# liuQuan98/APR

Measured on AMD Instinct MI355X. Metric: point-cloud pairs/sec (120k-pt KITTI frame, FCGF encode+match+SVD), higher is better.
Workload: dtype f32

## Files before the change

apr_amd/_lib.py:

```python
from __future__ import annotations

import ctypes as C
import os

import torch

_HERE = os.path.dirname(os.path.abspath(__file__))
LIB_PATH = os.path.join(_HERE, "lib", "libapr_hip.so")

_p = C.c_void_p
_i32, _i64, _u64, _f32, _f64, _sz = C.c_int32, C.c_int64, C.c_uint64, C.c_float, C.c_double, C.c_size_t

class PairDesc(C.Structure):
    _fields_ = [("f0", C.c_void_p), ("n0", C.c_int64), ("f1", C.c_void_p), ("n1", C.c_int64),
                ("xyz0", C.c_void_p), ("xyz1", C.c_void_p), ("seed", C.c_uint64)]


class SpconvDesc(C.Structure):
    _fields_ = [("inp", C.c_void_p), ("ldi", C.c_int64), ("nbr", C.c_void_p), ("n_out", C.c_int64),
                ("K", C.c_int32), ("cin", C.c_int32), ("cout", C.c_int32), ("relu", C.c_int32),
                ("w_packed", C.c_void_p), ("scale", C.c_void_p), ("shift", C.c_void_p),
                ("residual", C.c_void_p), ("ldr", C.c_int64), ("out", C.c_void_p), ("ldo", C.c_int64),
                ("counters", C.c_void_p), ("plist", C.c_void_p), ("prod_scratch", C.c_void_p),
                ("plist_bytes", C.c_int64), ("w_bf3", C.c_void_p),
# ... 63 lines not shown
    "apr_map_scratch_bytes": (_sz, [_i64]),
    "apr_voxelize": (C.c_int, [_p, _i64, _f32, _i32, _p, _p]),
    "apr_map_build": (C.c_int, [_p, _i64, _p, _i32, _p, _p, _i64, _p, _p, _p, _p, _p, _sz, _p]),
    "apr_kernel_map_transpose": (C.c_int, [_p, _i64, _i32, _i64, _p, _p]),
    "apr_voxelize_segments": (C.c_int, [_p, _i64, C.c_float, _p, _i32, _p, _p]),
    "apr_segment_counts": (C.c_int, [_p, _p, _p, _i32, _p, _p]),
    "apr_kernel_map_same": (C.c_int, [_p, _i64, _p, _p, _i64, _i32, _i32, _p, _p]),
    "apr_kernel_map": (C.c_int, [_p, _i64, _p, _p, _p, _i64, _i32, _i32, _p, _p]),
    "apr_spconv_packed_size": (_i64, [_i32, _i32, _i32]),
    "apr_spconv_pack_weights": (C.c_int, [_p, _i32, _i32, _i32, _p, _p]),
    "apr_spconv_fwd": (C.c_int, [_p, _i64, _p, _i64, _i32, _i32, _i32, _p, _p, _p, _p, _i64, _i32, _p, _i64, _p]),
    "apr_pairlist_counter_ints": (_i32, []),
    "apr_pairlist_bytes": (_sz, [_i64, _i32]),
    "apr_pairlist_build": (C.c_int, [_p, _i64, _i32, _p, _p, _sz, _p]),
    "apr_pairlist3_bytes": (_sz, [_i64]),
    "apr_pairlist3_build": (C.c_int, [_p, _i64, _i32, _p, _p, _sz, _p]),
    "apr_spconv_ws3_supported": (C.c_int, [_i32, _i32, _i32]),
    "apr_spconv_ws3_fwd_bf3": (C.c_int, [_p, _i64, _p, _p, _i64, _i32, _i32, _p, _p, _p, _p, _i64, _i32, _p, _i64, _p, _p]),
    "apr_spconv_ws_fwd": (C.c_int, [_p, _i64, _p, _p, _i64, _i32, _i32, _i32, _p, _p, _p, _p, _i64, _i32, _p, _i64, _p, _p]),
    "apr_spconv_packed_bf3_bytes": (_i64, [_i32, _i32, _i32]),
    "apr_spconv_pack_weights_bf3": (C.c_int, [_p, _i32, _i32, _i32, _p, _p]),
    "apr_spconv_pack_weights_bf3_ex": (C.c_int, [_p, _i32, _i32, _i32, _i32, _i32, _p, _p]),
    "apr_spconv_ws_fwd_bf3": (C.c_int, [_p, _i64, _p, _p, _i64, _i32, _i32, _i32, _p, _p, _p, _p, _p, _i64, _i32, _p, _i64,
                                        _p, _p]),
    "apr_spconv_wgrad_scratch_bytes": (_sz, [_i64, _i32, _i32, _i32]),
    "apr_spconv_wgrad": (C.c_int, [_p, _i64, _p, _i64, _p, _i64, _i32, _i32, _i32, _p, _p, _sz, _p]),
    "apr_spconv_wgrad_same_level": (C.c_int, [_p, _i64, _p, _i64, _p, _i64, _i32, _i32, _i32, _p, _p, _sz, _p]),
    "apr_spconv_route": (_i32, [_p]),
    "apr_spconv_ws_supported": (_i32, [_i32, _i32, _i32]),
    "apr_spconv_bigk_supported": (_i32, [_i32, _i32, _i32]),
    "apr_spconv_fwd_batch": (C.c_int, [_p, _i32, _p]),
    "apr_spconv_fwd_batch_timed": (C.c_int, [_p, _i32, _p, _p]),
    "apr_bn_stats": (C.c_int, [_p, _i64, _i64, _i32, _p, _p, _p, _sz, _p]),
    "apr_norm_params": (C.c_int, [_p, _i64, _i64, _i32, _f32, _p, _p, _p, _sz, _p]),
    "apr_bn_stats_scratch_bytes": (_sz, [_i64, _i32]),
    "apr_instance_norm_act": (C.c_int, [_p, _i64, _i64, _i32, _f32, _p, _i64, _i32, _f32, _p, _i64, _p, _sz, _p]),
    "apr_spconv_os_tile_rows": (_i32, [_i64, _i32, _i32]),
    "apr_spconv_os_pairs_bytes": (_sz, [_i64, _i32, _i32]),
    "apr_spconv_os_pairs_build": (C.c_int, [_p, _i64, _i64, _i32, _i32, _p, _sz, _p]),
    "apr_spconv_os_trace": (C.c_int, [_p, _i32]),
    "apr_spconv_os_set_debug": (C.c_int, [_i32]),
    "apr_spconv_os_fwd": (C.c_int, [_p, _i64, _p, _i64, _i32, _i32, _i32, _i32, _p, _p, _p, _p, _i64, _i32, _p, _i64, _p]),
    "apr_norm_backward_scratch_bytes": (_sz, [_i64, _i32]),
    "apr_norm_backward": (C.c_int, [_p, _i64, _p, _i64, _i64, _i32, _p, _p, _p, _p, _i64, _p, _p, _p, _sz, _p]),
    "apr_bn_train_fwd": (C.c_int, [_p, _i64, _i64, _i32, _p, _p, C.c_float, C.c_float, _p, _p, _p, _i64, _i32, _p, _i64, _p, _p,
                                   _p, _p, _i32, _p, _sz, _p]),
    "apr_bn_train_bwd": (C.c_int, [_p, _i64, _p, _i64, _p, _i64, _i64, _i32, _p, _p, _p, _i32, _p, _i64, _p, _i64, _p, _p,
                                   _p, _i32, _p, _sz, _p]),
    "apr_weights_flip_transpose": (C.c_int, [_p, _i32, _i32, _i32, _i32, _p, _p]),
    "apr_dense_gemm_bf3": (C.c_int, [_p, _i64, _i64, _i32, _i32, _p, _p, _p, _p, _i64, _i32, _p, _i64, _p]),
    "apr_dense_rows_bf3_ok": (_i32, [_i32, _i32]),
    "apr_dense_rows_bf3_route": (_i32, [_i64, _i32, _i32]),
    "apr_dense_rows_bf3": (C.c_int, [_p, _i64, _i64, _i32, _i32, _p, _p, _p, _p, _i64, _i32, _i32, _p, _i64, _p]),
    "apr_dense_gemm_bf3_norm_scratch_bytes": (_sz, [_i64, _i32, _i32]),
    "apr_dense_gemm_bf3_norm_act": (C.c_int, [_p, _i64, _i64, _i32, _i32, _p, _f32, _p, _i64, _i32, _f32, _p, _i64, _p, _i32, _p,
                                              _sz, _p]),
    "apr_weighted_choice_round": (C.c_int64, [_p, _i64, _p, _i64, _i64, _p, _i64, _p, _p, _i32]),
    "apr_instance_norm_act_seg": (C.c_int, [_p, _i64, _i64, _i32, _f32, _p, _i64, _i32, _f32, _p, _i64, _p, _i32, _p, _sz, _p]),
    "apr_affine_act": (C.c_int, [_p, _i64, _i64, _i32, _p, _p, _p, _i64, _i32, _f32, _p, _i64, _p]),
    "apr_act_backward": (C.c_int, [_p, _i64, _p, _i64, _i64, _i32, _i32, _f32, _p, _i64, _p]),
    "apr_l2_normalize": (C.c_int, [_p, _i64, _i64, _i32, _p, _i64, _p]),
    "apr_l2_normalize_backward": (C.c_int, [_p, _i64, _p, _i64, _i64, _i32, _p, _i64, _p]),
    "apr_feature_nn": (C.c_int, [_p, _i64, _p, _i64, _i32, _p, _p]),
    "apr_feature_nn_fast_scratch_bytes": (_sz, [_i64, _i64, _i32]),
    "apr_feature_nn_fast": (C.c_int, [_p, _i64, _p, _i64, _i32, _p, _p, _sz, _p]),
    "apr_nn_unpack": (C.c_int, [_p, _i64, _p, _p, _p]),
    "apr_ransac_scratch_bytes": (_sz, [_i64, _i64]),
    "apr_ransac_pose": (C.c_int, [_p, _i64, _p, _i64, _p, _f64, _f64, _i64, _u64, _p, _sz, _p, _p]),
    "apr_ransac_geometric_scratch_bytes": (_sz, [_i64, _i64, _i64]),
    "apr_ransac_pose_geometric": (C.c_int, [_p, _i64, _p, _i64, _p, _f64, _f64, _i64, _i64, _u64, _p, _sz, _p, _p]),
    "apr_ransac_raw_bytes": (_sz, []),
    "apr_ransac_pose_geometric_async": (C.c_int, [_p, _i64, _p, _i64, _p, _f64, _f64, _i64, _i64, _u64, _p, _sz, _p, _p]),
    "apr_ransac_decode": (C.c_int, [_p, _p]),
    "apr_ransac_pose_async": (C.c_int, [_p, _i64, _p, _i64, _p, _f64, _f64, _i64, _u64, _p, _sz, _p, _p]),
    "apr_fcgf_test_pair": (C.c_int, [_p, _i64, _p, _i64, _p, _p, _i64, _i64, _p, _p, _i64, _p, _i64, _p, _p, _p, _f64, _f64,
                                     _f64, _i64, _p, _p, _i64, _i64, _p]),
    "apr_irls_pose": (C.c_int, [_p, _p, _p, _i64, _p, _p, _sz, _p]),
    "apr_match_pose_batch_scratch_bytes": (_sz, [_i32, _i64, _i64, _i32, _i64]),
    "apr_match_pose_batch": (C.c_int, [_p, _i32, _i32, C.c_double, C.c_double, _i64, _p, _sz, _p, _p]),
    "apr_match_pose_batch_slot_bytes": (_sz, [_i32]),
    "apr_match_pose_set_lanes": (C.c_int, [_i32]),
    "apr_match_pose_batch_enqueue": (C.c_int, [_p, _i32, _i32, C.c_double, C.c_double, _i64, _p, _sz, _p, _p]),
    "apr_match_pose_batch_finish": (C.c_int, [_p, _i32, _i32, C.c_double, C.c_double, _i64, _p, _sz, _p, _p, _p]),
    "apr_irls_scratch_bytes": (_sz, [_i64]),
    "apr_valid_pair": (C.c_int, [_p, _i64, _p, _i64, _p, _p, _i64, _i64, _p, _p, _f32, _p, _i64, _i64, _p, _sz, _p]),
    "apr_valid_pair_scratch_bytes": (_sz, [_i64]),
    "apr_predator_valid_record": (C.c_int, [_p, _p, _p, _p, _p, _p, _p, _p, _i64, _i64, _p, _i64, _i64, _p]),
    "apr_predator_test_pair": (C.c_int, [_p, _i64, _p, _i64, _p, _p, _p, _p, _f64, _f64, _f64, _f64, _p, _i64, _i64, _p]),
    "apr_contrastive_reduce": (C.c_int, [_p, _p, _i32, _i32, _p, _p, _p, _p, _p, _p, _p, _i32, _i64, _f32, _f32, _p, _p]),
    "apr_pair_rows_from_nn": (C.c_int, [_p, _i64, _p, _i64, _p, _p]),
    "apr_pair_dist": (C.c_int, [_p, _i64, _p, _i64, _i32, _p, _p, _i64, _i64, _f32, _p, _p, _p, _p]),
    "apr_pair_terms_scratch_bytes": (_sz, [_i64]),
    "apr_pair_terms_reduce": (C.c_int, [_p, _p, _p, _i64, _p, _i64, _p, _i64, _i64, _f32, _i32, _p, _p, _p, _p, _p, _p, _sz, _p]),
    "apr_pair_grad_scratch_bytes": (_sz, [_i64, _i64, _i64]),
    "apr_pair_grad": (C.c_int, [_p, _i64, _p, _i64, _i32, _p, _p, _i64, _p, _p, _p, _p, _i32, _p, _p, _p, _sz, _p]),
    "apr_grid_subsample_scratch_bytes": (_sz, [_i64]),
    "apr_grid_subsample": (C.c_int, [_p, _i64, _p, _i32, _f32, _p, _i32, _p, _p, _p, _p, _sz, _p]),
    "apr_grid_subsample_async": (C.c_int, [_p, _i64, _p, _i32, _f32, _p, _i32, _p, _p, _p, _p, _sz, _p]),
    "apr_voxel_down_sample_scratch_bytes": (_sz, [_i64]),
    "apr_voxel_down_sample": (C.c_int, [_p, _i64, _p, _i32, _f64, _p, _p, _p, _p, _p, _p, _p, _sz, _p]),
    "apr_sample_augment": (C.c_int, [_p, _p, _i64, _f64, _p, _f64, _p, _p, _p]),
    "apr_cloud_mean": (C.c_int, [_p, _i64, _p, _p]),
    "apr_radius_scratch_bytes": (_sz, [_i64, _i64]),
    "apr_radius_neighbors_async": (C.c_int, [_p, _i64, _p, _i64, _p, _p, _i32, _f32, _i32, _p, _i64, _p, _p, _sz, _p]),
    "apr_radius_neighbors_regrid_async": (C.c_int, [_p, _i64, _p, _i64, _p, _p, _i32, _f32, _i32, _p, _i64, _p, _p, _sz, _p]),
    "apr_radius_neighbors": (C.c_int, [_p, _i64, _p, _i64, _p, _p, _i32, _f32, _i32, _p, _i64, _p, _p, _sz, _p]),
# ... 132 lines not shown
```

apr_amd/csrc/common.h:

```cpp
#pragma once
#include <hip/hip_runtime.h>
#include <stdint.h>
#include <stdio.h>
#include <stdlib.h>
#include <string.h>

#include "../../include/apr_hip.h"

static inline int env_int(const char* name, int dflt) {
  const char* v = getenv(name);
  return v ? atoi(v) : dflt;
}

#define APR_API extern "C" __attribute__((visibility("default")))

void apr_set_error(const char* fmt, ...);

#define APR_CHECK_ARG(cond, ...)      \
  do {                                \
    if (!(cond)) {                    \
      apr_set_error(__VA_ARGS__);     \
      return APR_EINVAL;              \
    }                                 \
  } while (0)

#define APR_HIP(call)                                                            \
  do {                                                                           \
    hipError_t e_ = (call);                                                      \
    if (e_ != hipSuccess) {                                                      \
      apr_set_error("%s:%d %s -> %s", __FILE__, __LINE__, #call, hipGetErrorString(e_)); \
      return APR_EHIP;                                                           \
    }                                                                            \
  } while (0)

#define APR_LAUNCH_CHECK() APR_HIP(hipGetLastError())

static inline int64_t cdiv64(int64_t a, int64_t b) { return (a + b - 1) / b; }

__host__ __device__ static inline size_t apr_align256(size_t x) { return (x + 255) & ~(size_t)255; }

struct AprArena {
  char* base;
  size_t off = 0;
  explicit AprArena(void* scratch) : base((char*)apr_align256((size_t)scratch)) {}
  template <typename T>
  T* take(size_t count) {
    T* p = base ? (T*)(base + off) : nullptr;
    off += apr_align256(count * sizeof(T));
    return p;
  }
  size_t bytes() const { return off + 256; }
  bool fits(size_t scratch_bytes) const { return scratch_bytes >= bytes(); }
};

int apr_internal_nn_brute(const float* f0, int64_t n0, const float* f1, int64_t n1, int32_t c, uint64_t* best,
                          const unsigned* run_if, void* stream);

int apr_internal_fill(void* ptr, int32_t byte_value, size_t bytes, hipStream_t st);

bool apr_internal_dense_ok(int64_t M, int32_t cin, int32_t cout);
bool apr_internal_dense_rows_route(int64_t M, int32_t cin, int32_t cout);
bool apr_internal_ws_bf3_only(const void* w_bf3, int32_t cin);
int apr_internal_dense_gemm(const float* in, int64_t ldi, int64_t M, int32_t cin, int32_t cout, const float* wp,
                            const float* scale, const float* shift, const float* residual, int64_t ldr, int32_t relu,
                            float* out, int64_t ldo, hipStream_t st);

bool apr_internal_spconv_bigk_aligned(const apr_spconv_desc& d);
int apr_internal_spconv_bigk(const apr_spconv_desc& d, hipStream_t st);

int apr_internal_norm_apply_partials(const float* x, int64_t ldx, int32_t c, const int64_t* seg_row0, const int* seg_blk0,
                                     int32_t nseg, const double* partial, float eps, const float* residual, int64_t ldr,
                                     int32_t act_mode, float negative_slope, float* y, int64_t ldy, hipStream_t st);

#ifdef __HIPCC__
__device__ inline int apr_wave_incl_scan(int x) {
  x += __builtin_amdgcn_update_dpp(0, x, 0x111, 0xf, 0xf, true);
  x += __builtin_amdgcn_update_dpp(0, x, 0x112, 0xf, 0xf, true);
  x += __builtin_amdgcn_update_dpp(0, x, 0x114, 0xf, 0xf, true);
  x += __builtin_amdgcn_update_dpp(0, x, 0x118, 0xf, 0xf, true);
  x += __builtin_amdgcn_update_dpp(0, x, 0x142, 0xa, 0xf, true);
  x += __builtin_amdgcn_update_dpp(0, x, 0x143, 0xc, 0xf, true);
  return x;
}
#endif

#define APR_KEY_EMPTY 0xFFFFFFFFFFFFFFFFull
#define APR_AXIS_BIAS (1 << 17)
#define APR_AXIS_RANGE (1 << 18)

__host__ __device__ static inline bool apr_key_in_range(int b, int x, int y, int z) {
  return (unsigned)b < 1023u && (unsigned)(x + APR_AXIS_BIAS) < (unsigned)APR_AXIS_RANGE &&
         (unsigned)(y + APR_AXIS_BIAS) < (unsigned)APR_AXIS_RANGE &&
         (unsigned)(z + APR_AXIS_BIAS) < (unsigned)APR_AXIS_RANGE;
}

__host__ __device__ static inline uint64_t apr_pack_key(int b, int x, int y, int z) {
  return ((((uint64_t)(unsigned)b << 18 | (uint64_t)(unsigned)(x + APR_AXIS_BIAS)) << 18 |
           (uint64_t)(unsigned)(y + APR_AXIS_BIAS))
          << 18) |
         (uint64_t)(unsigned)(z + APR_AXIS_BIAS);
}

__host__ __device__ static inline uint32_t apr_hash_u64(uint64_t k) {
  k ^= k >> 33;
  k *= 0xff51afd7ed558ccdull;
  k ^= k >> 33;
  k *= 0xc4ceb9fe1a85ec53ull;
  k ^= k >> 33;
  return (uint32_t)k;
}

__host__ __device__ static inline int apr_floor_to(int v, int m) {
  int q = v / m;
  if ((v % m) != 0 && v < 0) --q;
// ... 52 lines not shown
```

apr_amd/csrc/dense_rows.hip:

```cpp
#include "common.h"
#include "bf3.h"
#include <mutex>

namespace {

typedef float f32x4 __attribute__((ext_vector_type(4)));

constexpr int kRowsWaves = 8;
constexpr int kRowsTile = kRowsWaves * 32;

template <int NSTEP, int NC>
__global__ __launch_bounds__(64 * kRowsWaves, 1) void k_dense_rows_bf3(
    const float* __restrict__ in, int64_t ldi, int M, const unsigned char* __restrict__ wp3,
    const float* __restrict__ scale, const float* __restrict__ shift, const float* __restrict__ residual, int64_t ldr,
    int relu, int l2norm, float* __restrict__ out, int64_t ldo, int ntile) {
  extern __shared__ __attribute__((aligned(16))) unsigned char s_w[];
  constexpr int G = 2;
  constexpr int NB64 = (NC + 3) / 4;
  constexpr int kPlane = NSTEP * 4096;
  constexpr int kImage = NB64 * 3 * kPlane;
  const int tid = threadIdx.x, lane = tid & 63;
  const int wave = __builtin_amdgcn_readfirstlane(tid >> 6);
  const int r16 = lane & 15, q = lane >> 4;
  const int frag_off = (r16 * 4 + ((r16 & 8) ? (q ^ 3) : q)) * 16;
// ... 99 lines not shown
        for (int cb = 0; cb < NS; ++cb)
#pragma unroll
          for (int e = 0; e < 4; ++e) {
            sq[cb][e] = fmaf(v[cb][e], v[cb][e], 0.f);
            if (NC >= 8) sq[cb][e] = fmaf(v[cb + 4][e], v[cb + 4][e], sq[cb][e]);
          }
#pragma unroll
        for (int d = NS / 2; d >= 1; d >>= 1)
#pragma unroll
          for (int cb = 0; cb < d; ++cb) sq[cb] += sq[cb + d];
        f32x4 s = sq[0];
#pragma unroll
        for (int e = 0; e < 4; ++e) s[e] += __shfl_xor(s[e], 32);
#pragma unroll
        for (int e = 0; e < 4; ++e) s[e] += __shfl_xor(s[e], 16);
        const float nrm = sqrtf((s[0] + s[2]) + (s[1] + s[3]));
#pragma unroll
        for (int cb = 0; cb < NC; ++cb) {
          v[cb][0] = v[cb][0] / nrm; v[cb][1] = v[cb][1] / nrm; v[cb][2] = v[cb][2] / nrm; v[cb][3] = v[cb][3] / nrm;
        }
      }
      if (live) {
#pragma unroll
        for (int cb = 0; cb < NC; ++cb)
          *reinterpret_cast<f32x4*>(out + (int64_t)r * ldo + cb * 16 + q * 4) = v[cb];
      }
    }
  }
}

template <int NSTEP, int NC>
int launch_rows(const float* in, int64_t ldi, int64_t M, const void* w_bf3, const float* scale, const float* shift,
                const float* residual, int64_t ldr, int relu, int l2norm, float* out, int64_t ldo, hipStream_t st) {
  constexpr int kImage = ((NC + 3) / 4) * 3 * NSTEP * 4096;
  constexpr int kAffBytes = 2 * NC * 16 * 4;
  static_assert(kImage + kAffBytes <= 160 * 1024, "weight image does not fit the LDS");
  auto kern = k_dense_rows_bf3<NSTEP, NC>;
  {
    static std::mutex s_mu;
    static bool s_attr[64] = {};
    int dev = 0;
    APR_HIP(hipGetDevice(&dev));
    std::lock_guard<std::mutex> lk(s_mu);
    if (dev >= 0 && dev < 64 && !s_attr[dev]) {
      APR_HIP(hipFuncSetAttribute((const void*)kern, hipFuncAttributeMaxDynamicSharedMemorySize, kImage + kAffBytes));
      s_attr[dev] = true;
    }
  }
  const int ntile = (int)cdiv64(M, kRowsTile);
  static const int s_grid = env_int("APR_DENSE_ROWS_GRID", 256);
  const int grid = ntile < s_grid ? ntile : s_grid;
  hipLaunchKernelGGL(kern, dim3((unsigned)grid), dim3(64 * kRowsWaves), kImage + kAffBytes, st, in, ldi, (int)M,
                     (const unsigned char*)w_bf3, scale, shift, residual, ldr, relu, l2norm, out, ldo, ntile);
  APR_LAUNCH_CHECK();
  return APR_OK;
}

}

APR_API int32_t apr_dense_rows_bf3_ok(int32_t cin, int32_t cout) {
  if (cin % 32 != 0 || cin < 64 || cin > 192) return 0;
  if (cout != 32 && cout != 64 && cout != 128) return 0;
  return (((cout + 63) / 64) * 3 * (cin / 32) * 4096 + 8 * cout <= 160 * 1024) ? 1 : 0;
}

bool apr_internal_dense_rows_route(int64_t M, int32_t cin, int32_t cout) {
  static const int s_min = env_int("APR_DENSE_ROWS_MIN", 32768);
  return s_min > 0 && M >= s_min && apr_dense_rows_bf3_ok(cin, cout);
}

APR_API int32_t apr_dense_rows_bf3_route(int64_t M, int32_t cin, int32_t cout) {
  return apr_internal_dense_rows_route(M, cin, cout) ? 1 : 0;
}

APR_API int apr_dense_rows_bf3(const float* in, int64_t ldi, int64_t M, int32_t cin, int32_t cout, const void* w_bf3,
                               const float* scale, const float* shift, const float* residual, int64_t ldr, int32_t relu,
                               int32_t l2norm, float* out, int64_t ldo, void* stream) {
  APR_CHECK_ARG(in && out && w_bf3 && M > 0 && M < (1ll << 31) - kRowsTile && apr_dense_rows_bf3_ok(cin, cout),
                "apr_dense_rows_bf3: needs M > 0, cin in 64..192 step 32, cout 32 / 64 / 128 (got %d -> %d)", cin, cout);
  APR_CHECK_ARG(ldi >= cin && ldo >= cout && ldi % 4 == 0 && ldo % 4 == 0 && ((uintptr_t)in & 15) == 0 &&
                    ((uintptr_t)out & 15) == 0,
                "apr_dense_rows_bf3: rows of in / out must be 16-byte aligned");
  APR_CHECK_ARG(!residual || (ldr >= cout && ldr % 4 == 0 && ((uintptr_t)residual & 15) == 0),
                "apr_dense_rows_bf3: residual rows must be 16-byte aligned");
  APR_CHECK_ARG((!scale || ((uintptr_t)scale & 15) == 0) && (!shift || ((uintptr_t)shift & 15) == 0),
                "apr_dense_rows_bf3: scale / shift must be 16-byte aligned");
  hipStream_t st = (hipStream_t)stream;
#define APR_ROWS_CASE(NS, NCB)                                                                                       \
  if (cin == NS * 32 && cout == NCB * 16)                                                                            \
    return launch_rows<NS, NCB>(in, ldi, M, w_bf3, scale, shift, residual, ldr, relu, l2norm, out, ldo, st);
  APR_ROWS_CASE(2, 2) APR_ROWS_CASE(2, 4) APR_ROWS_CASE(2, 8)
  APR_ROWS_CASE(3, 2) APR_ROWS_CASE(3, 4) APR_ROWS_CASE(3, 8)
  APR_ROWS_CASE(4, 2) APR_ROWS_CASE(4, 4) APR_ROWS_CASE(4, 8)
  APR_ROWS_CASE(5, 2) APR_ROWS_CASE(5, 4) APR_ROWS_CASE(5, 8)
  APR_ROWS_CASE(6, 2) APR_ROWS_CASE(6, 4) APR_ROWS_CASE(6, 8)
#undef APR_ROWS_CASE
  apr_set_error("apr_dense_rows_bf3: no instantiation for %d -> %d", cin, cout);
  return APR_EINVAL;
}
```

apr_amd/csrc/encoder.hip:

```cpp
#include "common.h"

namespace {

constexpr int kLevels = 4, kStages = 7, kMaps = 10, kMaxLists = 24;

struct ListSlot {
  int map, kind, rows;
  void* blob;
  size_t bytes;
  int32_t* counters;
  bool built;
};

struct Enc {
  const apr_resunet_plan& P;
  const apr_level_map* lv;
  const int32_t* bbox;
  AprArena arena;
  const bool dry;
  hipStream_t st;
  int rc = APR_OK;

  int32_t* kmap[kMaps] = {};
  ListSlot lists[kMaxLists];
// ... 173 lines not shown
      n_counter_slots = 16;
      counters = arena.take<int32_t>((size_t)n_counter_slots * apr_pairlist_counter_ints());
      if (!dry) run(apr_fill_bytes(counters, 0, (size_t)n_counter_slots * apr_pairlist_counter_ints() * 4, st));
    }
    if (!dry) prod = (float*)arena.take<char>(prod_bytes_live);

    const int ch1 = L[0].cout, ch2 = L[3].cout, ch3 = L[6].cout, ch4 = L[9].cout;
    const int tr4 = L[12].cout, tr3 = L[15].cout, tr2 = L[18].cout;
    const int w1 = tr2 + ch1, w2 = tr3 + ch2, w3 = tr4 + ch3;
    float* cat1 = rows(n[0], w1);
    float* cat2 = rows(n[1], w2);
    float* cat3 = rows(n[2], w3);
    float* s8 = rows(n[3], ch4);
    int64_t amax = 0;
    {
      const int64_t c[kStages] = {n[0] * ch1, n[1] * ch2, n[2] * ch3, n[3] * ch4, n[2] * tr4, n[1] * tr3, n[0] * tr2};
      for (int s = 0; s < kStages; ++s) amax = c[s] > amax ? c[s] : amax;
    }
    float* A = arena.take<float>((size_t)amax);
    float* H = arena.take<float>((size_t)amax);
    float* h1 = rows(n[0], L[21].cout);

    struct StageIo {
      const float* in; int64_t ldi; int cmap, bmap, lout; float* out; int64_t ldo;
    };
    const StageIo io[kStages] = {
        {nullptr, 0, -1, 0, 0, cat1 + tr2, w1},
        {cat1 + tr2, w1, 4, 1, 1, cat2 + tr3, w2},
        {cat2 + tr3, w2, 5, 2, 2, cat3 + tr4, w3},
        {cat3 + tr4, w3, 6, 3, 3, s8, ch4},
        {s8, ch4, 9, 2, 2, cat3, w3},
        {cat3, w3, 8, 1, 1, cat2, w2},
        {cat2, w2, 7, 0, 0, cat1, w1},
    };
    for (int s = 0; s < kStages && ok(); ++s) {
      const apr_resunet_layer &C = L[3 * s], &B1 = L[3 * s + 1], &B2 = L[3 * s + 2];
      const StageIo& q = io[s];
      const int64_t n_out = n[q.lout];
      if (s == 0) {
        if (!dry)
          run(apr_occ_conv(lv[0].coords, n_out, bbox, P.conv1_ks, P.conv1_w, C.cout, C.scale, C.shift, nullptr, 0, C.relu, A,
                           C.cout, occ, occ_bytes + 256, st));
      } else {
        ListSlot* cl = ((P.ws_conv >> s) & 1u) && apr_spconv_ws_supported(C.K, C.cin, C.cout) ? ws_list(C, q.cmap, false) : nullptr;
        conv(C, q.in, q.ldi, q.cmap, n_out, cl, nullptr, 0, A, C.cout, false);
      }
      ListSlot* bl = nullptr;
      if (((P.os_block >> s) & 1u) && B1.cin == 64 && B1.w_bf3 && n_out >= P.os_min_rows) bl = os_list(B1, q.bmap);
      if (!bl && ((P.ws_block >> s) & 1u) && apr_spconv_ws_supported(B1.K, B1.cin, B1.cout)) bl = ws_list(B1, q.bmap, true);
      conv(B1, A, B1.cin, q.bmap, n_out, bl, nullptr, 0, H, B1.cout, false);
      conv(B2, H, B2.cin, q.bmap, n_out, bl, A, B1.cin, q.out, q.ldo, false);
      flush();
    }
    conv(L[21], cat1, w1, -1, n[0], nullptr, nullptr, 0, h1, L[21].cout, false);
    conv(L[22], h1, L[21].cout, -1, n[0], nullptr, nullptr, 0, out, ldo, P.normalize != 0);
    flush();
  }
  size_t prod_bytes_live = 0;
};

bool plan_ok(const apr_resunet_plan* p, const apr_level_map* lv, const int32_t* bbox) {
  if (!p || !lv || !bbox || !p->conv1_w) return false;
  for (int l = 0; l < kLevels; ++l)
    if (lv[l].n <= 0 || !lv[l].coords || !lv[l].keys || !lv[l].vals || lv[l].cap <= 0 || (lv[l].cap & (lv[l].cap - 1))) return false;
  for (int i = 0; i < 23; ++i)
    if (!p->layer[i].w_packed || p->layer[i].cin <= 0 || p->layer[i].cout <= 0) return false;
  for (int i = 1; i < 21; ++i)
    if (p->layer[i].K != 27) return false;
  if (p->layer[21].K != 1 || p->layer[22].K != 1) return false;
  const apr_resunet_layer* L = p->layer;
  for (int s = 0; s < kStages; ++s)
    if (L[3 * s + 1].cin != L[3 * s].cout || L[3 * s + 1].cout != L[3 * s].cout || L[3 * s + 2].cin != L[3 * s].cout ||
        L[3 * s + 2].cout != L[3 * s].cout)
      return false;
  if (L[3].cin != L[0].cout || L[6].cin != L[3].cout || L[9].cin != L[6].cout || L[12].cin != L[9].cout ||
      L[15].cin != L[12].cout + L[6].cout || L[18].cin != L[15].cout + L[3].cout || L[21].cin != L[18].cout + L[0].cout ||
      L[22].cin != L[21].cout)
    return false;
  if (L[0].cin != 1 || L[0].K != p->conv1_ks * p->conv1_ks * p->conv1_ks || L[0].cout % 8 != 0) return false;
  if (p->conv1_ks != 3 && p->conv1_ks != 5 && p->conv1_ks != 7) return false;
  return true;
}

}

APR_API int apr_resunet_encode_supported(const apr_resunet_plan* plan, const apr_level_map* lv, const int32_t* bbox_host) {
  if (!plan_ok(plan, lv, bbox_host)) return 0;
  return apr_occ_conv_pays(bbox_host, plan->conv1_ks, lv[0].n) ? 1 : 0;
}

APR_API size_t apr_resunet_encode_scratch_bytes(const apr_resunet_plan* plan, const apr_level_map* lv, const int32_t* bbox_host) {
  if (!apr_resunet_encode_supported(plan, lv, bbox_host)) return 0;
  Enc e(*plan, lv, bbox_host, nullptr, nullptr);
  e.walk(nullptr, plan->layer[22].cout);
  return e.need();
}

APR_API int apr_resunet_encode(const apr_resunet_plan* plan, const apr_level_map* lv, const int32_t* bbox_host, int32_t* counters,
                               int32_t n_counter_slots, void* scratch, size_t scratch_bytes, float* out, int64_t ldo,
                               void* stream) {
  APR_CHECK_ARG(apr_resunet_encode_supported(plan, lv, bbox_host),
                "apr_resunet_encode: plan / maps / box not covered (apr_resunet_encode_supported)");
  APR_CHECK_ARG(scratch && out && ldo >= plan->layer[22].cout && (!counters || n_counter_slots > 0),
                "apr_resunet_encode: bad arguments");
  Enc dry(*plan, lv, bbox_host, nullptr, nullptr);
  dry.walk(nullptr, ldo);
  APR_CHECK_ARG(scratch_bytes >= dry.need(), "apr_resunet_encode: scratch too small");
  Enc e(*plan, lv, bbox_host, scratch, (hipStream_t)stream);
  e.counters = counters;
// ... 105 lines not shown
```

apr_amd/ops.py:

```python
from __future__ import annotations

import ctypes as C
import os

import numpy as np
import torch

from . import _lib
from ._lib import check, ptr, stream


def _lib_():
    return _lib.load()


def _f32(t, name):
    if not t.is_cuda or t.dtype != torch.float32:
        raise _lib.AprHipError(f"{name}: need a float32 GPU tensor (no CPU fallback), got {t.dtype} on {t.device}")
    return t


def _rows(t, name):
    _f32(t, name)
    if t.dim() != 2 or (t.shape[1] > 1 and t.stride(1) != 1):
# ... 608 lines not shown
        return lib.apr_dense_rows_bf3(d.inp, d.ldi, d.n_out, d.cin, d.cout, d.w_bf3, *epi, 0, d.out, d.ldo, st)
    if route == _lib.ROUTE_DENSE_GEMM:
        return lib.apr_dense_gemm_bf3(d.inp, d.ldi, d.n_out, d.cin, d.cout, d.w_bf3, *epi, d.out, d.ldo, st)
    return lib.apr_spconv_fwd(d.inp, d.ldi, d.nbr, d.n_out, d.K, d.cin, d.cout, d.w_packed, *epi, d.out, d.ldo, st)


def spconv(x, nbr, K, cin, cout, wp, scale=None, shift=None, residual=None, relu=False, out=None, n_out=None,
           plist=None, w_bf3=None, os_pairs=None):
    prof = PROFILE
    if prof is not None and nbr is None:
        w_bf3 = None
    d, route, out, lst, _keep = _spconv_desc(x, nbr, K, cin, cout, wp, scale, shift, residual, relu, out, n_out, plist, w_bf3,
                                             os_pairs, {})
    if lst is not None:
        if lst.queued:
            raise _lib.AprHipError("spconv: the pair lists of this map are queued for building in a SpconvBatch that has not "
                                   "been launched yet")
        lst.build()
    if route == _lib.ROUTE_OS:
        prof = None
    if prof is not None:
        P = prof.pairs(nbr, d.n_out)
        e0, e1 = torch.cuda.Event(enable_timing=True), torch.cuda.Event(enable_timing=True)
        e0.record()
    check(_launch_routed(_lib_(), route, d, stream()))
    if prof is not None:
        e1.record()
        prof.records.append((P, cin, cout, K <= 32 and cin % 32 == 0 and cout % 32 == 0, e0, e1, _route_label(route)))
    return out


def dense_rows_bf3(x, w_bf3, cin, cout, scale=None, shift=None, residual=None, relu=False, l2norm=False, out=None):
    x, ldi = _rows(x, "dense_rows_bf3.x")
    if x.shape[1] != cin:
        raise _lib.AprHipError(f"dense_rows_bf3: input has {x.shape[1]} channels, weight expects {cin}")
    n = x.shape[0]
    if out is None:
        out = torch.empty((n, cout), dtype=torch.float32, device=x.device)
    out, ldo = _rows(out, "dense_rows_bf3.out")
    if out.shape[0] != n or out.shape[1] != cout:
        raise _lib.AprHipError("dense_rows_bf3: output shape mismatch")
    ldr = 0
    if residual is not None:
        residual, ldr = _rows(residual, "dense_rows_bf3.residual")
        if residual.shape[0] != n or residual.shape[1] != cout:
            raise _lib.AprHipError("dense_rows_bf3: residual shape mismatch")
    if n == 0:
        return out
    check(_lib_().apr_dense_rows_bf3(ptr(x), ldi, n, cin, cout, ptr(w_bf3), ptr(scale), ptr(shift), ptr(residual), ldr,
                                     int(bool(relu)), int(bool(l2norm)), ptr(out), ldo, stream()))
    return out


def dense_gemm_bf3(x, w_bf3, cin, cout, scale=None, shift=None, residual=None, relu=False, out=None):
    x, ldi = _rows(x, "dense_gemm_bf3.x")
    if x.shape[1] != cin:
        raise _lib.AprHipError(f"dense_gemm_bf3: input has {x.shape[1]} channels, weight expects {cin}")
    n = x.shape[0]
    if out is None:
        out = torch.empty((n, cout), dtype=torch.float32, device=x.device)
    out, ldo = _rows(out, "dense_gemm_bf3.out")
    ldr = 0
    if residual is not None:
        residual, ldr = _rows(residual, "dense_gemm_bf3.residual")
    check(_lib_().apr_dense_gemm_bf3(ptr(x), ldi, n, cin, cout, ptr(w_bf3), ptr(scale), ptr(shift), ptr(residual), ldr,
                                     int(bool(relu)), ptr(out), ldo, stream()))
    return out


WGRAD_PAD = os.environ.get("APR_WGRAD_PAD", "1") != "0"


def weights_flip_transpose(w, flip):
    w = _f32(w.detach(), "weights_flip_transpose.w").contiguous()
    K, cin, cout = w.shape
    wt = torch.empty((K, cout, cin), dtype=torch.float32, device=w.device)
    check(_lib_().apr_weights_flip_transpose(ptr(w), K, cin, cout, int(bool(flip)), ptr(wt), stream()))
    return wt


def spconv_wgrad(x, dout, nbr, K, cin, cout, same_level=False):
    if x.shape[1] != cin or dout.shape[1] != cout:
        raise _lib.AprHipError("spconv_wgrad: channel mismatch")
    if (cin % 32 or cout % 32) and WGRAD_PAD and x.shape[0] * (-cin % 32) + dout.shape[0] * (-cout % 32) < (1 << 26):
        cp, op = (cin + 31) // 32 * 32, (cout + 31) // 32 * 32
        xp = torch.nn.functional.pad(x, (0, cp - cin)) if cp != cin else x
        dp = torch.nn.functional.pad(dout, (0, op - cout)) if op != cout else dout
        return spconv_wgrad(xp, dp, nbr, K, cp, op, same_level=same_level)[:, :cin, :cout]
    x, ldi = _rows(x, "spconv_wgrad.x")
    dout, ldo = _rows(dout, "spconv_wgrad.dout")
    n_out = dout.shape[0]
    if nbr is not None and (nbr.dtype != torch.int32 or not nbr.is_contiguous() or tuple(nbr.shape) != (n_out, K)):
        raise _lib.AprHipError("spconv_wgrad: nbr must be a contiguous int32 [n_out, K] tensor")
    lib = _lib_()
    dw = torch.empty((K, cin, cout), dtype=torch.float32, device=x.device)
    sb = int(lib.apr_spconv_wgrad_scratch_bytes(n_out, K, cin, cout))
    scratch = torch.empty(sb, dtype=torch.uint8, device=x.device)
    fn = lib.apr_spconv_wgrad_same_level if (same_level and nbr is not None) else lib.apr_spconv_wgrad
    check(fn(ptr(x), ldi, ptr(dout), ldo, ptr(nbr), n_out, K, cin, cout, ptr(dw), ptr(scratch), sb, stream()))
    return dw


def _seg_array(segments, n):
    if segments is None or len(segments) <= 2:
        return None, 0
    if int(segments[0]) != 0 or int(segments[-1]) != n:
# ... 1190 lines not shown
```

include/apr_hip.h:

```cpp
#ifndef APR_HIP_H
#define APR_HIP_H

#include <stddef.h>
#include <stdint.h>

#ifdef __cplusplus
extern "C" {
#endif

#define APR_OK 0
#define APR_EINVAL (-1)
#define APR_EHIP (-2)
#define APR_ETIMEOUT (-3)
#define APR_ERANGE (-3)

const char* apr_last_error(void);
int apr_version(void);
int apr_device_count(void);
int32_t apr_struct_sizes(int32_t* out, int32_t n);
int apr_event_wait(void* event, int32_t poll_us);
int apr_event_wait_timeout(void* event, int32_t poll_us, int64_t timeout_us);


int64_t apr_hash_capacity(int64_t n);
// ... 318 lines not shown
                          int64_t n_terms, const int64_t* sorted_pos_keys, int64_t n_keys, int64_t hash_seed, float margin,
                          int32_t n_groups, double* red, float* mean, float* coef, int32_t* grp, uint8_t* kept,
                          void* scratch, size_t scratch_bytes, void* stream);
size_t apr_pair_grad_scratch_bytes(int64_t n, int64_t N0, int64_t N1);
int apr_pair_grad(const float* F0, int64_t N0, const float* F1, int64_t N1, int32_t c, const int32_t* r0, const int32_t* r1,
                  int64_t n, const float* coef, const int32_t* grp, const double* red, const float* gout, int32_t n_gout,
                  float* dF0, float* dF1, void* scratch, size_t scratch_bytes, void* stream);


size_t apr_grid_subsample_scratch_bytes(int64_t n);
int apr_grid_subsample(const float* pts, int64_t n, const int32_t* lengths_host, int32_t nb, float dl,
                       const float* feats, int32_t fdim, float* out_pts, float* out_feats,
                       int32_t* out_lengths_host, void* scratch, size_t scratch_bytes, void* stream);
int apr_grid_subsample_async(const float* pts, int64_t n, const int32_t* lengths_host, int32_t nb, float dl,
                             const float* feats, int32_t fdim, float* out_pts, float* out_feats,
                             int32_t* lengths_status_dev, void* scratch, size_t scratch_bytes, void* stream);

size_t apr_voxel_down_sample_scratch_bytes(int64_t n);
int apr_voxel_down_sample(const float* pts, int64_t n, const int32_t* lengths_host, int32_t nb, double voxel_size,
                          double* centroid, float* centroid32, int32_t* count, int32_t* first, int32_t* index,
                          int32_t* out_lengths_host, void* scratch, size_t scratch_bytes, void* stream);

int apr_sample_augment(const double* pts, const double* u, int64_t n, double noise, const double* rot_host,
                       double scale, const double* shift_host, float* out, void* stream);

int apr_cloud_mean(const float* pts, int64_t n, double* mean, void* stream);

size_t apr_radius_scratch_bytes(int64_t nq, int64_t ns);
int apr_radius_neighbors(const float* queries, int64_t nq, const float* supports, int64_t ns,
                         const int32_t* q_lengths_host, const int32_t* s_lengths_host, int32_t nb, float radius,
                         int32_t limit, int32_t* out, int64_t out_ld, int32_t* width_host,
                         void* scratch, size_t scratch_bytes, void* stream);

int apr_radius_neighbors_async(const float* queries, int64_t nq, const float* supports, int64_t ns,
                               const int32_t* q_lengths_host, const int32_t* s_lengths_host, int32_t nb, float radius,
                               int32_t limit, int32_t* out, int64_t out_ld, int32_t* flags_dev,
                               void* scratch, size_t scratch_bytes, void* stream);
int apr_radius_neighbors_regrid_async(const float* queries, int64_t nq, const float* supports, int64_t ns,
                               const int32_t* q_lengths_host, const int32_t* s_lengths_host, int32_t nb, float radius,
                               int32_t limit, int32_t* out, int64_t out_ld, int32_t* flags_dev,
                               void* scratch, size_t scratch_bytes, void* stream);

int apr_knn(const float* pts, int32_t n, int32_t k, int32_t skip_first, int32_t* out, void* stream);


int apr_dense_gemm_bf3(const float* in, int64_t ldi, int64_t M, int32_t cin, int32_t cout, const void* w_bf3,
                       const float* scale, const float* shift, const float* residual, int64_t ldr, int32_t relu,
                       float* out, int64_t ldo, void* stream);
int32_t apr_dense_rows_bf3_ok(int32_t cin, int32_t cout);
int32_t apr_dense_rows_bf3_route(int64_t M, int32_t cin, int32_t cout);
int apr_dense_rows_bf3(const float* in, int64_t ldi, int64_t M, int32_t cin, int32_t cout, const void* w_bf3,
                       const float* scale, const float* shift, const float* residual, int64_t ldr, int32_t relu,
                       int32_t l2norm, float* out, int64_t ldo, void* stream);
size_t apr_dense_gemm_bf3_norm_scratch_bytes(int64_t M, int32_t cout, int32_t nseg);
int apr_dense_gemm_bf3_norm_act(const float* in, int64_t ldi, int64_t M, int32_t cin, int32_t cout, const void* w_bf3,
                                float eps, const float* residual, int64_t ldr, int32_t act_mode, float negative_slope,
                                float* out, int64_t ldo, const int64_t* seg_offsets_host, int32_t nseg, void* scratch,
                                size_t scratch_bytes, void* stream);

typedef struct apr_kp_resnet_desc {
  const float* x; int64_t ldx; int64_t n_in;
  int32_t in_dim, mid, out_dim, strided;
  const float* q_pts; const float* s_pts; int64_t n_out;
  const int32_t* nbr; int32_t H; int32_t n_kp;
  const float* kernel_points; float extent; float eps; float slope; int32_t nseg;
  const void* w_unary1; const void* w_kpconv; const void* w_unary2; const void* w_shortcut;
  const int64_t* seg_in; const int64_t* seg_out;
  float* out; int64_t ldo;
  void* scratch; size_t scratch_bytes;
  int32_t kpconv_route;
} apr_kp_resnet_desc;
size_t apr_kp_resnet_scratch_bytes(const apr_kp_resnet_desc* desc);
int apr_kp_resnet_block(const apr_kp_resnet_desc* desc, void* stream);

int64_t apr_weighted_choice_round(double* p, int64_t n, int64_t* found, int64_t n_uniq, int64_t n_new_zeroed,
                                  const double* x, int64_t k, double* cdf, int32_t* stamp, int32_t round_id);

int apr_row_sums(const float* x, int64_t ld, int64_t n, int32_t c, float* out, void* stream);

int apr_kpconv_weighted(const float* q_pts, int64_t nq, const float* s_pts, int64_t ns, const int32_t* nbr,
                        int32_t H, const float* x, int64_t ldx, int32_t cin, const float* kernel_points,
                        int32_t n_kp, float extent, const float* rowsum, float* wf, int64_t ldwf, void* stream);
int32_t apr_kpconv_fused_ok(int32_t cin, int32_t cout, int32_t H);
int32_t apr_kpconv_fused_route(int64_t nq, int32_t cin, int32_t cout, int32_t H);
int apr_kpconv_fused(const float* q_pts, int64_t nq, const float* s_pts, int64_t ns, const int32_t* nbr, int32_t H,
                     const float* x, int64_t ldx, int32_t cin, const float* kernel_points, int32_t n_kp, float extent,
                     const float* rowsum, const void* w_bf3, int32_t cout, float* out, int64_t ldo, void* stream);
int apr_kpconv_dfeat(const float* q_pts, int64_t nq, const float* s_pts, int64_t ns, const int32_t* nbr, int32_t H,
                     const float* dwf, int64_t lddwf, int32_t cin, const float* kernel_points, int32_t n_kp,
                     float extent, const float* rowsum, float* dx, int64_t lddx, void* stream);

int apr_kpconv_dfeat_contrib(const float* q_pts, int64_t nq, const float* s_pts, int64_t ns, const int32_t* nbr, int32_t H,
                             const float* dwf, int64_t lddwf, int32_t cin, const float* kernel_points, int32_t n_kp,
                             float extent, const float* rowsum, float* contrib, void* stream);
int apr_kpconv_deform_weighted(const float* q_pts, int64_t nq, const float* s_pts, int64_t ns, const int32_t* nbr, int32_t H,
                               const float* x, int64_t ldx, int32_t cin, const float* dkp, const float* mod, int32_t n_kp,
                               float extent, const float* rowsum, float* wf, int64_t ldwf, float* min_d2, void* stream);
int apr_kpconv_deform_dfeat_contrib(const float* q_pts, int64_t nq, const float* s_pts, int64_t ns, const int32_t* nbr,
                                    int32_t H, const float* dwf, int64_t lddwf, int32_t cin, const float* dkp, const float* mod,
                                    int32_t n_kp, float extent, const float* rowsum, float* contrib, void* stream);
int apr_kpconv_deform_dgeom(const float* q_pts, int64_t nq, const float* s_pts, int64_t ns, const int32_t* nbr, int32_t H,
                            const float* x, int64_t ldx, int32_t cin, const float* dwf, int64_t lddwf, const float* dkp,
                            const float* mod, int32_t n_kp, float extent, const float* rowsum, float* d_dkp, float* d_mod,
                            void* stream);
size_t apr_reverse_table_scratch_bytes(int64_t nq, int32_t H, int64_t ns);
int apr_reverse_table_build(const int32_t* nbr, int64_t nq, int32_t H, int64_t ns, int32_t* rev_t, int32_t* start,
// ... 162 lines not shown
```

Before: 2810.

## Fuse final two 1x1 encoder layers into one dense rows kernel

Adds a kernel that runs the last two pointwise layers of the encoder (96->64->32, with affine, ReLU and optional L2 normalisation) in one pass, keeping the intermediate activations in LDS instead of writing them to global memory. The encoder tail uses it when the shapes, bf16x3 weights and alignment match, and otherwise falls back to the two separate convs. This removes one launch and the round trip of the 64-wide intermediate tensor. In exchange it uses a large LDS footprint with one block per CU, and its route depends on the existing rows-route heuristics.

```diff
diff --git a/apr_amd/_lib.py b/apr_amd/_lib.py
--- a/apr_amd/_lib.py
+++ b/apr_amd/_lib.py
@@ -139,6 +139,8 @@
     "apr_dense_rows_bf3_ok": (_i32, [_i32, _i32]),
     "apr_dense_rows_bf3_route": (_i32, [_i64, _i32, _i32]),
     "apr_dense_rows_bf3": (C.c_int, [_p, _i64, _i64, _i32, _i32, _p, _p, _p, _p, _i64, _i32, _i32, _p, _i64, _p]),
+    "apr_dense_rows2_bf3_ok": (_i32, [_i32, _i32, _i32]),
+    "apr_dense_rows2_bf3": (C.c_int, [_p, _i64, _i64, _i32, _i32, _i32, _p, _p, _p, _i32, _p, _p, _p, _i32, _i32, _p, _i64, _p]),
     "apr_dense_gemm_bf3_norm_scratch_bytes": (_sz, [_i64, _i32, _i32]),
     "apr_dense_gemm_bf3_norm_act": (C.c_int, [_p, _i64, _i64, _i32, _i32, _p, _f32, _p, _i64, _i32, _f32, _p, _i64, _p, _i32, _p,
                                               _sz, _p]),
diff --git a/apr_amd/csrc/common.h b/apr_amd/csrc/common.h
--- a/apr_amd/csrc/common.h
+++ b/apr_amd/csrc/common.h
@@ -60,6 +60,7 @@
 
 bool apr_internal_dense_ok(int64_t M, int32_t cin, int32_t cout);
 bool apr_internal_dense_rows_route(int64_t M, int32_t cin, int32_t cout);
+bool apr_internal_dense_rows2_route(int64_t M, int32_t cin, int32_t mid, int32_t cout);
 bool apr_internal_ws_bf3_only(const void* w_bf3, int32_t cin);
 int apr_internal_dense_gemm(const float* in, int64_t ldi, int64_t M, int32_t cin, int32_t cout, const float* wp,
                             const float* scale, const float* shift, const float* residual, int64_t ldr, int32_t relu,
diff --git a/apr_amd/csrc/dense_rows.hip b/apr_amd/csrc/dense_rows.hip
--- a/apr_amd/csrc/dense_rows.hip
+++ b/apr_amd/csrc/dense_rows.hip
@@ -175,6 +175,225 @@
   const int grid = ntile < s_grid ? ntile : s_grid;
   hipLaunchKernelGGL(kern, dim3((unsigned)grid), dim3(64 * kRowsWaves), kImage + kAffBytes, st, in, ldi, (int)M,
                      (const unsigned char*)w_bf3, scale, shift, residual, ldr, relu, l2norm, out, ldo, ntile);
+  APR_LAUNCH_CHECK();
+  return APR_OK;
+}
+
+template <int NSTEP, int NC1, int NC2>
+__global__ __launch_bounds__(64 * kRowsWaves, 1) void k_dense_rows2_bf3(
+    const float* __restrict__ in, int64_t ldi, int M, const unsigned char* __restrict__ wp3a,
+    const unsigned char* __restrict__ wp3b, const float* __restrict__ scale1, const float* __restrict__ shift1, int relu1,
+    const float* __restrict__ scale2, const float* __restrict__ shift2, int relu2, int l2norm, float* __restrict__ out,
+    int64_t ldo, int ntile) {
+  extern __shared__ __attribute__((aligned(16))) unsigned char s_w[];
+  constexpr int G = 2;
+  constexpr int NSTEP2 = NC1 / 2;
+  static_assert(NC1 % 2 == 0 && NC2 <= 4, "intermediate width: a multiple of 32; output: up to 64 columns");
+  constexpr int kPlane1 = NSTEP * 4096, kImage1 = ((NC1 + 3) / 4) * 3 * kPlane1;
+  constexpr int kPlane2 = NSTEP2 * 4096, kImage2 = ((NC2 + 3) / 4) * 3 * kPlane2;
+  constexpr int kAff = (NC1 + NC2) * 16;
+  constexpr int LDT = NC1 * 16 + 4;
+  const int tid = threadIdx.x, lane = tid & 63;
+  const int wave = __builtin_amdgcn_readfirstlane(tid >> 6);
+  const int r16 = lane & 15, q = lane >> 4;
+  const int frag_off = (r16 * 4 + ((r16 & 8) ? (q ^ 3) : q)) * 16;
+  unsigned char* s_w2 = s_w + kImage1;
+  float* s_aff = reinterpret_cast<float*>(s_w + kImage1 + kImage2);
+  float* s_t = s_aff + 2 * kAff + wave * (G * 16 * LDT);
+
+  int t = blockIdx.x;
+  const float* arow[G];
+#pragma unroll
+  for (int gi = 0; gi < G; ++gi) {
+    const int r = t * kRowsTile + wave * 32 + gi * 16 + r16;
+    arow[gi] = in + (int64_t)(r < M ? r : M - 1) * ldi + q * 8;
+  }
+  f32x4 abuf[G][NSTEP][2];
+#pragma unroll
+  for (int s = 0; s < NSTEP; ++s)
+#pragma unroll
+    for (int gi = 0; gi < G; ++gi) {
+      abuf[gi][s][0] = __builtin_nontemporal_load(reinterpret_cast<const f32x4*>(arow[gi] + s * 32));
+      abuf[gi][s][1] = __builtin_nontemporal_load(reinterpret_cast<const f32x4*>(arow[gi] + s * 32 + 4));
+    }
+  for (int c = wave; c < kImage1 / 1024; c += kRowsWaves)
+    __builtin_amdgcn_global_load_lds((const __attribute__((address_space(1))) void*)(wp3a + (int64_t)c * 1024 + lane * 16),
+                                     (__attribute__((address_space(3))) void*)(s_w + c * 1024), 16, 0, 0);
+  for (int c = wave; c < kImage2 / 1024; c += kRowsWaves)
+    __builtin_amdgcn_global_load_lds((const __attribute__((address_space(1))) void*)(wp3b + (int64_t)c * 1024 + lane * 16),
+                                     (__attribute__((address_space(3))) void*)(s_w2 + c * 1024), 16, 0, 0);
+  if (tid < NC1 * 16) {
+    s_aff[tid] = scale1 ? scale1[tid] : 1.f;
+    s_aff[kAff + tid] = shift1 ? shift1[tid] : 0.f;
+  } else if (tid < kAff) {
+    const int c = tid - NC1 * 16;
+    s_aff[tid] = scale2 ? scale2[c] : 1.f;
+    s_aff[kAff + tid] = shift2 ? shift2[c] : 0.f;
+  }
+  asm volatile("s_waitcnt vmcnt(0)" ::: "memory");
+  __syncthreads();
+
+  for (; t < ntile; t += gridDim.x) {
+    const int tn = t + gridDim.x;
+    const bool more = tn < ntile;
+    const float* nrow[G];
+#pragma unroll
+    for (int gi = 0; gi < G; ++gi) {
+      const int64_t r = (int64_t)tn * kRowsTile + wave * 32 + gi * 16 + r16;
+      nrow[gi] = in + (r < M ? r : (int64_t)M - 1) * ldi + q * 8;
+    }
+    f32x4 acc[G][NC1];
+#pragma unroll
+    for (int gi = 0; gi < G; ++gi)
+#pragma unroll
+      for (int cb = 0; cb < NC1; ++cb) acc[gi][cb] = (f32x4){0.f, 0.f, 0.f, 0.f};
+    int woff = frag_off, coff = q * 4;
+    asm volatile("" : "+v"(woff), "+v"(coff));
+
+#define APR_ROWS_MFMA(ACC, W, A)                                                                                     \
+  _Pragma("unroll") for (int gi = 0; gi < G; ++gi)                                                                   \
+    ACC[gi][cb] = __builtin_amdgcn_mfma_f32_16x16x32_bf16(W, A[gi], ACC[gi][cb], 0, 0, 0);
+#pragma unroll
+    for (int s = 0; s < NSTEP; ++s) {
+      bf16x8 ah[G], am[G], al[G];
+#pragma unroll
+      for (int gi = 0; gi < G; ++gi) apr_split3(abuf[gi][s][0], abuf[gi][s][1], ah[gi], am[gi], al[gi]);
+      if (more) {
+#pragma unroll
+        for (int gi = 0; gi < G; ++gi) {
+          abuf[gi][s][0] = __builtin_nontemporal_load(reinterpret_cast<const f32x4*>(nrow[gi] + s * 32));
+          abuf[gi][s][1] = __builtin_nontemporal_load(reinterpret_cast<const f32x4*>(nrow[gi] + s * 32 + 4));
+        }
+      }
+#pragma unroll
+      for (int cb = 0; cb < NC1; ++cb) {
+        const unsigned char* wb = s_w + (cb >> 2) * (3 * kPlane1) + s * 4096 + (cb & 3) * 1024 + woff;
+        const bf16x8 wh = *reinterpret_cast<const bf16x8*>(wb);
+        const bf16x8 wm = *reinterpret_cast<const bf16x8*>(wb + kPlane1);
+        const bf16x8 wl = *reinterpret_cast<const bf16x8*>(wb + 2 * kPlane1);
+        APR_ROWS_MFMA(acc, wl, ah) APR_ROWS_MFMA(acc, wh, al) APR_ROWS_MFMA(acc, wm, am)
+        APR_ROWS_MFMA(acc, wm, ah) APR_ROWS_MFMA(acc, wh, am) APR_ROWS_MFMA(acc, wh, ah)
+      }
+    }
+#pragma unroll
+    for (int gi = 0; gi < G; ++gi) {
+#pragma clang fp contract(off)
+#pragma unroll
+      for (int cb = 0; cb < NC1; ++cb) {
+        const f32x4 sc = *reinterpret_cast<const f32x4*>(s_aff + cb * 16 + coff);
+        const f32x4 sh = *reinterpret_cast<const f32x4*>(s_aff + kAff + cb * 16 + coff);
+        f32x4 a = acc[gi][cb] * sc;
+        a = a + sh;
+        if (relu1) {
+          a[0] = fmaxf(a[0], 0.f); a[1] = fmaxf(a[1], 0.f); a[2] = fmaxf(a[2], 0.f); a[3] = fmaxf(a[3], 0.f);
+        }
+        *reinterpret_cast<f32x4*>(s_t + (gi * 16 + r16) * LDT + cb * 16 + coff) = a;
+      }
+    }
+    __builtin_amdgcn_fence(__ATOMIC_RELEASE, "wavefront");
+    __builtin_amdgcn_wave_barrier();
+    __builtin_amdgcn_fence(__ATOMIC_ACQUIRE, "wavefront");
+
+    f32x4 acc2[G][NC2];
+#pragma unroll
+    for (int gi = 0; gi < G; ++gi)
+#pragma unroll
+      for (int cb = 0; cb < NC2; ++cb) acc2[gi][cb] = (f32x4){0.f, 0.f, 0.f, 0.f};
+#pragma unroll
+    for (int s = 0; s < NSTEP2; ++s) {
+      bf16x8 ah[G], am[G], al[G];
+#pragma unroll
+      for (int gi = 0; gi < G; ++gi) {
+        const float* hr = s_t + (gi * 16 + r16) * LDT + s * 32 + 2 * coff;
+        apr_split3(*reinterpret_cast<const f32x4*>(hr), *reinterpret_cast<const f32x4*>(hr + 4), ah[gi], am[gi], al[gi]);
+      }
+#pragma unroll
+      for (int cb = 0; cb < NC2; ++cb) {
+        const unsigned char* wb = s_w2 + (cb >> 2) * (3 * kPlane2) + s * 4096 + (cb & 3) * 1024 + woff;
+        const bf16x8 wh = *reinterpret_cast<const bf16x8*>(wb);
+        const bf16x8 wm = *reinterpret_cast<const bf16x8*>(wb + kPlane2);
+        const bf16x8 wl = *reinterpret_cast<const bf16x8*>(wb + 2 * kPlane2);
+        APR_ROWS_MFMA(acc2, wl, ah) APR_ROWS_MFMA(acc2, wh, al) APR_ROWS_MFMA(acc2, wm, am)
+        APR_ROWS_MFMA(acc2, wm, ah) APR_ROWS_MFMA(acc2, wh, am) APR_ROWS_MFMA(acc2, wh, ah)
+      }
+    }
+#undef APR_ROWS_MFMA
+    __builtin_amdgcn_fence(__ATOMIC_RELEASE, "wavefront");
+    __builtin_amdgcn_wave_barrier();
+
+#pragma unroll
+    for (int gi = 0; gi < G; ++gi) {
+      const int r = t * kRowsTile + wave * 32 + gi * 16 + r16;
+      const bool live = r < M;
+      f32x4 v[NC2];
+      {
+#pragma clang fp contract(off)
+#pragma unroll
+        for (int cb = 0; cb < NC2; ++cb) {
+          const f32x4 sc = *reinterpret_cast<const f32x4*>(s_aff + NC1 * 16 + cb * 16 + coff);
+          const f32x4 sh = *reinterpret_cast<const f32x4*>(s_aff + kAff + NC1 * 16 + cb * 16 + coff);
+          f32x4 a = acc2[gi][cb] * sc;
+          a = a + sh;
+          if (relu2) {
+            a[0] = fmaxf(a[0], 0.f); a[1] = fmaxf(a[1], 0.f); a[2] = fmaxf(a[2], 0.f); a[3] = fmaxf(a[3], 0.f);
+          }
+          v[cb] = a;
+        }
+      }
+      if (l2norm) {
+        f32x4 sq[NC2];
+#pragma unroll
+        for (int cb = 0; cb < NC2; ++cb)
+#pragma unroll
+          for (int e = 0; e < 4; ++e) sq[cb][e] = fmaf(v[cb][e], v[cb][e], 0.f);
+#pragma unroll
+        for (int d = NC2 / 2; d >= 1; d >>= 1)
+#pragma unroll
+          for (int cb = 0; cb < d; ++cb) sq[cb] += sq[cb + d];
+        f32x4 s = sq[0];
+#pragma unroll
+        for (int e = 0; e < 4; ++e) s[e] += __shfl_xor(s[e], 32);
+#pragma unroll
+        for (int e = 0; e < 4; ++e) s[e] += __shfl_xor(s[e], 16);
+        const float nrm = sqrtf((s[0] + s[2]) + (s[1] + s[3]));
+#pragma unroll
+        for (int cb = 0; cb < NC2; ++cb) {
+          v[cb][0] = v[cb][0] / nrm; v[cb][1] = v[cb][1] / nrm; v[cb][2] = v[cb][2] / nrm; v[cb][3] = v[cb][3] / nrm;
+        }
+      }
+      if (live) {
+#pragma unroll
+        for (int cb = 0; cb < NC2; ++cb)
+          *reinterpret_cast<f32x4*>(out + (int64_t)r * ldo + cb * 16 + q * 4) = v[cb];
+      }
+    }
+  }
+}
+
+template <int NSTEP, int NC1, int NC2>
+int launch_rows2(const float* in, int64_t ldi, int64_t M, const void* wa, const void* wb, const float* scale1,
+                 const float* shift1, int relu1, const float* scale2, const float* shift2, int relu2, int l2norm, float* out,
+                 int64_t ldo, hipStream_t st) {
+  constexpr int kImage1 = ((NC1 + 3) / 4) * 3 * NSTEP * 4096, kImage2 = ((NC2 + 3) / 4) * 3 * (NC1 / 2) * 4096;
+  constexpr int kLds = kImage1 + kImage2 + 2 * (NC1 + NC2) * 16 * 4 + kRowsWaves * 2 * 16 * (NC1 * 16 + 4) * 4;
+  static_assert(kLds <= 160 * 1024, "the two weight images and the patches do not fit the LDS");
+  auto kern = k_dense_rows2_bf3<NSTEP, NC1, NC2>;
+  {
+    static std::mutex s_mu;
+    static bool s_attr[64] = {};
+    int dev = 0;
+    APR_HIP(hipGetDevice(&dev));
+    std::lock_guard<std::mutex> lk(s_mu);
+    if (dev >= 0 && dev < 64 && !s_attr[dev]) {
+      APR_HIP(hipFuncSetAttribute((const void*)kern, hipFuncAttributeMaxDynamicSharedMemorySize, kLds));
+      s_attr[dev] = true;
+    }
+  }
+  const int ntile = (int)cdiv64(M, kRowsTile);
+  static const int s_grid = env_int("APR_DENSE_ROWS_GRID", 256);
+  const int grid = ntile < s_grid ? ntile : s_grid;
+  hipLaunchKernelGGL(kern, dim3((unsigned)grid), dim3(64 * kRowsWaves), kLds, st, in, ldi, (int)M, (const unsigned char*)wa,
+                     (const unsigned char*)wb, scale1, shift1, relu1, scale2, shift2, relu2, l2norm, out, ldo, ntile);
   APR_LAUNCH_CHECK();
   return APR_OK;
 }
@@ -221,3 +440,27 @@
   apr_set_error("apr_dense_rows_bf3: no instantiation for %d -> %d", cin, cout);
   return APR_EINVAL;
 }
+
+APR_API int32_t apr_dense_rows2_bf3_ok(int32_t cin, int32_t mid, int32_t cout) {
+  return (cin == 96 && mid == 64 && cout == 32) ? 1 : 0;
+}
+
+bool apr_internal_dense_rows2_route(int64_t M, int32_t cin, int32_t mid, int32_t cout) {
+  static const int s_on = env_int("APR_DENSE_ROWS2", 1);
+  return s_on && apr_dense_rows2_bf3_ok(cin, mid, cout) && apr_internal_dense_rows_route(M, cin, mid) &&
+         apr_internal_dense_rows_route(M, mid, cout);
+}
+
+APR_API int apr_dense_rows2_bf3(const float* in, int64_t ldi, int64_t M, int32_t cin, int32_t mid, int32_t cout,
+                                const void* w1_bf3, const float* scale1, const float* shift1, int32_t relu1,
+                                const void* w2_bf3, const float* scale2, const float* shift2, int32_t relu2, int32_t l2norm,
+                                float* out, int64_t ldo, void* stream) {
+  APR_CHECK_ARG(in && out && w1_bf3 && w2_bf3 && M > 0 && M < (1ll << 31) - kRowsTile && apr_dense_rows2_bf3_ok(cin, mid, cout),
+                "apr_dense_rows2_bf3: needs M > 0 and 96 -> 64 -> 32 channels (got %d -> %d -> %d)", cin, mid, cout);
+  APR_CHECK_ARG(ldi >= cin && ldo >= cout && ldi % 4 == 0 && ldo % 4 == 0 && ((uintptr_t)in & 15) == 0 &&
+                    ((uintptr_t)out & 15) == 0,
+                "apr_dense_rows2_bf3: rows of in / out must be 16-byte aligned");
+  APR_CHECK_ARG((((uintptr_t)w1_bf3 | (uintptr_t)w2_bf3) & 15) == 0, "apr_dense_rows2_bf3: weight images must be 16-byte aligned");
+  return launch_rows2<3, 4, 2>(in, ldi, M, w1_bf3, w2_bf3, scale1, shift1, relu1, scale2, shift2, relu2, l2norm, out, ldo,
+                               (hipStream_t)stream);
+}
diff --git a/apr_amd/csrc/encoder.hip b/apr_amd/csrc/encoder.hip
--- a/apr_amd/csrc/encoder.hip
+++ b/apr_amd/csrc/encoder.hip
@@ -249,9 +249,22 @@
       conv(B2, H, B2.cin, q.bmap, n_out, bl, A, B1.cin, q.out, q.ldo, false);
       flush();
     }
-    conv(L[21], cat1, w1, -1, n[0], nullptr, nullptr, 0, h1, L[21].cout, false);
-    conv(L[22], h1, L[21].cout, -1, n[0], nullptr, nullptr, 0, out, ldo, P.normalize != 0);
-    flush();
+    const apr_resunet_layer &T1 = L[21], &T2 = L[22];
+    bool tail2 = T1.K == 1 && T2.K == 1 && T1.w_bf3 && T2.w_bf3 && T2.cin == T1.cout &&
+                 apr_internal_dense_rows2_route(n[0], T1.cin, T1.cout, T2.cout);
+    if (tail2 && !dry)
+      tail2 = w1 % 4 == 0 && ldo % 4 == 0 &&
+              ((((uintptr_t)cat1) | ((uintptr_t)out) | ((uintptr_t)T1.scale) | ((uintptr_t)T1.shift) | ((uintptr_t)T2.scale) |
+                ((uintptr_t)T2.shift) | ((uintptr_t)T1.w_bf3) | ((uintptr_t)T2.w_bf3)) & 15) == 0;
+    if (tail2) {
+      if (!dry && ok())
+        run(apr_dense_rows2_bf3(cat1, w1, n[0], T1.cin, T1.cout, T2.cout, T1.w_bf3, T1.scale, T1.shift, T1.relu, T2.w_bf3,
+                                T2.scale, T2.shift, T2.relu, P.normalize != 0, out, ldo, st));
+    } else {
+      conv(T1, cat1, w1, -1, n[0], nullptr, nullptr, 0, h1, T1.cout, false);
+      conv(T2, h1, T1.cout, -1, n[0], nullptr, nullptr, 0, out, ldo, P.normalize != 0);
+      flush();
+    }
   }
   size_t prod_bytes_live = 0;
 };
diff --git a/apr_amd/ops.py b/apr_amd/ops.py
--- a/apr_amd/ops.py
+++ b/apr_amd/ops.py
@@ -684,6 +684,25 @@
     return out
 
 
+def dense_rows2_bf3(x, w1_bf3, w2_bf3, cin, mid, cout, scale1=None, shift1=None, relu1=False, scale2=None, shift2=None,
+                    relu2=False, l2norm=False, out=None):
+    x, ldi = _rows(x, "dense_rows2_bf3.x")
+    if x.shape[1] != cin:
+        raise _lib.AprHipError(f"dense_rows2_bf3: input has {x.shape[1]} channels, weight expects {cin}")
+    n = x.shape[0]
+    if out is None:
+        out = torch.empty((n, cout), dtype=torch.float32, device=x.device)
+    out, ldo = _rows(out, "dense_rows2_bf3.out")
+    if out.shape[0] != n or out.shape[1] != cout:
+        raise _lib.AprHipError("dense_rows2_bf3: output shape mismatch")
+    if n == 0:
+        return out
+    check(_lib_().apr_dense_rows2_bf3(ptr(x), ldi, n, cin, mid, cout, ptr(w1_bf3), ptr(scale1), ptr(shift1), int(bool(relu1)),
+                                      ptr(w2_bf3), ptr(scale2), ptr(shift2), int(bool(relu2)), int(bool(l2norm)), ptr(out),
+                                      ldo, stream()))
+    return out
+
+
 def dense_gemm_bf3(x, w_bf3, cin, cout, scale=None, shift=None, residual=None, relu=False, out=None):
     x, ldi = _rows(x, "dense_gemm_bf3.x")
     if x.shape[1] != cin:
diff --git a/include/apr_hip.h b/include/apr_hip.h
--- a/include/apr_hip.h
+++ b/include/apr_hip.h
@@ -394,6 +394,10 @@
 int apr_dense_rows_bf3(const float* in, int64_t ldi, int64_t M, int32_t cin, int32_t cout, const void* w_bf3,
                        const float* scale, const float* shift, const float* residual, int64_t ldr, int32_t relu,
                        int32_t l2norm, float* out, int64_t ldo, void* stream);
+int32_t apr_dense_rows2_bf3_ok(int32_t cin, int32_t mid, int32_t cout);
+int apr_dense_rows2_bf3(const float* in, int64_t ldi, int64_t M, int32_t cin, int32_t mid, int32_t cout, const void* w1_bf3,
+                        const float* scale1, const float* shift1, int32_t relu1, const void* w2_bf3, const float* scale2,
+                        const float* shift2, int32_t relu2, int32_t l2norm, float* out, int64_t ldo, void* stream);
 size_t apr_dense_gemm_bf3_norm_scratch_bytes(int64_t M, int32_t cout, int32_t nseg);
 int apr_dense_gemm_bf3_norm_act(const float* in, int64_t ldi, int64_t M, int32_t cin, int32_t cout, const void* w_bf3,
                                 float eps, const float* residual, int64_t ldr, int32_t act_mode, float negative_slope,
```

Result: slower. 2753 (-2.0%).
